# roiponytch/Flickering_Adversarial_Video

Hardware: AMD Instinct MI355X
Metric: attack-iters/sec (I3D 64x224x224, bs=8 per GPU; clip attack-iterations per second, whole job) + 3D-conv TFLOP/s (higher is better)
Workload: dtype bf16; 1 GPU; I3D-RGB flickering attack iteration (1 fwd + 1 dgrad bwd + Adam), 64x224x224 clips, bs=8 per GPU; global_batch=8, frames=64, parallelism=single, collective=none

## Files before the change

flickering_adversarial_video_amd/csrc/pool.hip:

```cpp
#include <stdlib.h>
#include <string.h>
#include "flk_internal.h"
#include "conv_common.h"

#ifdef FLK_ABLATE
#define PF_DBG(bit) (p.dbg & (bit))
#define PG_DBG(bit) (pg.dbg & (bit))
#else
#define PF_DBG(bit) (0)
#define PG_DBG(bit) (0)
#endif

struct PoolKP {
  const char* in; char* out; uint8_t* idx;
  const char* gout; char* gin; const char* mask; const char* add;
  int in_ld, in_coff, out_ld, out_coff, C;
  int gout_ld, gout_coff, gin_ld, gin_coff, mask_ld, mask_coff;
  int B, Ti, Hi, Wi, To, Ho, Wo;
  int kt, kh, kw, st, sh, sw, pt, ph, pw;
  int relu_input;
};

template <typename T> struct PV;
template <> struct PV<bf16_t> {
// ... 793 lines not shown

  frag8 af[KS][2];
  {
    const char* wp = pg.wpack + ((size_t)cslab * KS * 2 * 64 + lane) * 16;
#pragma unroll
    for (int ks = 0; ks < KS; ++ks)
#pragma unroll
      for (int f = 0; f < 2; ++f) af[ks][f] = *(const frag8*)(wp + (size_t)(ks * 2 + f) * 1024);
  }
  auto decode = [&](int hp, size_t& opos, int& lt0, int& lh0, int& lw0) {
    const int a = (int)(((float)hp + 0.5f) * inv_hw), rem = hp - a * nhw;
    const int bq = (int)(((float)rem + 0.5f) * inv_w), c = rem - bq * nw;
    const int ot = o_t0 + a, oh = o_h0 + bq, ow = o_w0 + c;
    opos = (((size_t)(b * k.To + ot) * k.Ho + oh) * k.Wo + ow);
    lt0 = ot * k.st - k.pt - i_t0; lh0 = oh * k.sh - k.ph - i_h0; lw0 = ow * k.sw - k.pw - i_w0;
  };
  auto product = [&](size_t opos, f32x4 (&v)[2]) {
    const char* gp = pg.g + (opos * pg.g_ld + pg.g_coff + q * 8) * 2;
    frag8 bf[KS];
#pragma unroll
    for (int ks = 0; ks < KS; ++ks) bf[ks] = *(const frag8*)(gp + ks * 64);
    v[0] = f32x4{0.f, 0.f, 0.f, 0.f}; v[1] = v[0];
#pragma unroll
    for (int ks = 0; ks < KS; ++ks) {
      v[0] = __builtin_amdgcn_mfma_f32_16x16x32_bf16(af[ks][0], bf[ks], v[0], 0, 0, 0);
      v[1] = __builtin_amdgcn_mfma_f32_16x16x32_bf16(af[ks][1], bf[ks], v[1], 0, 0, 0);
    }
  };
  __syncthreads();
  unsigned mx = 0u;
  for (int base = wave * 16; base < P; base += 64) {
    const int hp = min(base + m, P - 1);
    size_t opos; int lt0, lh0, lw0;
    decode(hp, opos, lt0, lh0, lw0);
    f32x4 v[2];
    product(opos, v);
#pragma unroll
    for (int f = 0; f < 2; ++f)
#pragma unroll
      for (int j = 0; j < 4; ++j) mx = max(mx, __float_as_uint(v[f][j]) & 0x7fffffffu);
  }
#pragma unroll
  for (int off = 32; off > 0; off >>= 1) mx = max(mx, (unsigned)__shfl_xor((int)mx, off));
  if (lane == 0) atomicMax(smax, mx);
  __syncthreads();
  int ex = (int)(*smax >> 23);
  ex = min(max(ex, 26), 254);
  const float scale = __uint_as_float((unsigned)(127 + p.fx_e + 127 - ex) << 23);
  const float inv_scale = __uint_as_float((unsigned)(127 - p.fx_e - 127 + ex) << 23);
  const int khkw = k.kh * k.kw;
  for (int base = wave * 16; base < P; base += 64) {
    const int hp = min(base + m, P - 1);
    const bool live = base + m < P;
    size_t opos; int lt0, lh0, lw0;
    decode(hp, opos, lt0, lh0, lw0);
    unsigned ib[2];
#pragma unroll
    for (int f = 0; f < 2; ++f) ib[f] = *(const unsigned*)(k.idx + opos * k.C + cslab * 32 + f * 16 + q * 4);
    f32x4 v[2];
    product(opos, v);
    if (!live) continue;
#pragma unroll
    for (int f = 0; f < 2; ++f)
#pragma unroll
      for (int j = 0; j < 4; ++j) {
        const int tap = (int)((ib[f] >> (8 * j)) & 255u);
        const int dt = (int)(((unsigned)tap * m_khkw) >> 20), r2 = tap - dt * khkw;
        const int dh = (int)(((unsigned)r2 * m_kw) >> 20), dw = r2 - dh * k.kw;
        const int lt = lt0 + dt, lh = lh0 + dh, lw = lw0 + dw;
        if ((unsigned)lt < (unsigned)p.Tt && (unsigned)lh < (unsigned)p.Ht && (unsigned)lw < (unsigned)p.Wt && dt < k.kt)
          atomicAdd(&acc[(f * 16 + q * 4 + j) * RS + (lt * p.Ht + lh) * p.Wt + lw], (unsigned)__float2int_rn(v[f][j] * scale));
      }
  }
  __syncthreads();
  const int ch = tid & 3, c0 = cslab * 32 + ch * 8;
  if (c0 >= k.C) return;
  const int hw = p.Ht * p.Wt;
  for (int r = tid >> 2; r < p.rows; r += 64) {
    int rt, rh, rw; split3(r, hw, 1.0f / (float)hw, p.Wt, 1.0f / (float)p.Wt, rt, rh, rw);
    const int it = i_t0 + rt, ih = i_h0 + rh, iw = i_w0 + rw;
    if (it >= k.Ti || ih >= k.Hi || iw >= k.Wi) continue;
    float g[8];
#pragma unroll
    for (int e = 0; e < 8; ++e) g[e] = (float)(int)acc[(ch * 8 + e) * RS + r] * inv_scale;
    const size_t ipos = (((size_t)(b * k.Ti + it) * k.Hi + ih) * k.Wi + iw);
    PV<bf16_t>::st(k.gin + (ipos * k.gin_ld + k.gin_coff + c0) * 2, g);
  }
}

template <int KS, int NIT, int NB>
__global__ __launch_bounds__(256, KS >= 3 ? 2 : 3) void maxpool_scatter_gemm_bwd_reg(const PoolGemmP pg, unsigned m_khkw, unsigned m_kw) {
  typedef __bf16 frag8 __attribute__((ext_vector_type(8)));
  extern __shared__ __attribute__((aligned(16))) char smem[];
  unsigned* const acc = (unsigned*)smem;
  const PoolTP& p = pg.t;
  const PoolKP& k = p.k;
  const int RS = p.plane_b;
  const int tid = threadIdx.x, lane = tid & 63, wave = tid >> 6, q = lane >> 4, m = lane & 15;
  int bid, cslab;
  if (!tile_slab_of_block(p, bid, cslab)) return;
  const int tw = bid % p.nTw; bid /= p.nTw;
  const int th = bid % p.nTh; bid /= p.nTh;
  const int tt = bid % p.nTt;
  const int b = bid / p.nTt;
  const int i_t0 = tt * p.Tt, i_h0 = th * p.Ht, i_w0 = tw * p.Wt;
  const int o_t0 = max(0, (i_t0 + k.pt - k.kt + k.st) / k.st), o_t1 = min(k.To - 1, (i_t0 + p.Tt - 1 + k.pt) / k.st);
  const int o_h0 = max(0, (i_h0 + k.ph - k.kh + k.sh) / k.sh), o_h1 = min(k.Ho - 1, (i_h0 + p.Ht - 1 + k.ph) / k.sh);
  const int o_w0 = max(0, (i_w0 + k.pw - k.kw + k.sw) / k.sw), o_w1 = min(k.Wo - 1, (i_w0 + p.Wt - 1 + k.pw) / k.sw);
  const int nt = max(0, o_t1 - o_t0 + 1), nh = max(0, o_h1 - o_h0 + 1), nw = max(0, o_w1 - o_w0 + 1);
  const int nhw = nh * nw, P = nt * nhw;
  const float inv_hw = 1.0f / (float)max(nhw, 1), inv_w = 1.0f / (float)max(nw, 1);
  if (!PG_DBG(16)) for (int i = tid; i < 32 * RS; i += 256) acc[i] = 0u;
  unsigned* const smax = acc + 32 * RS;
  if (tid == 0) *smax = 0u;
  unsigned* const lut = smax + 64;
  {
    const int dt = tid / 9, r2 = tid - dt * 9, dh = r2 / 3, dw = r2 - dh * 3;
    lut[tid] = tid < 27 ? (unsigned)(((dt * p.Ht + dh) * p.Wt + dw) * 4) : 0u;
  }
  f32x4 v[NIT][2];
  unsigned ib[NIT][2];
  int org[NIT];
  unsigned okm[NIT];
  unsigned mx = 0u;
  if (P > 0) {
    frag8 af[KS][2];
    {
      const char* wp = pg.wpack + ((size_t)cslab * KS * 2 * 64 + lane) * 16;
#pragma unroll
      for (int ks = 0; ks < KS; ++ks)
#pragma unroll
        for (int f = 0; f < 2; ++f) af[ks][f] = *(const frag8*)(wp + (size_t)(ks * 2 + f) * 1024);
    }
#pragma unroll
    for (int i0 = 0; i0 < NIT; i0 += NB) {
      frag8 bf[NB][KS];
#pragma unroll
      for (int u = 0; u < NB; ++u) {
        const int i = i0 + u;
        const int hp = wave * 16 + 64 * i + m;
        const bool live = hp < P;
        const int hc = min(hp, P - 1);
        const int a = (int)(((float)hc + 0.5f) * inv_hw), rem = hc - a * nhw;
        const int bq = (int)(((float)rem + 0.5f) * inv_w), c = rem - bq * nw;
        const int ot = o_t0 + a, oh = o_h0 + bq, ow = o_w0 + c;
        const size_t opos = (((size_t)(b * k.To + ot) * k.Ho + oh) * k.Wo + ow);
        const int lt0 = ot * k.st - k.pt - i_t0, lh0 = oh * k.sh - k.ph - i_h0, lw0 = ow * k.sw - k.pw - i_w0;
        org[i] = ((lt0 * p.Ht + lh0) * p.Wt + lw0) * 4;
        auto bits3 = [](int l0, int n) { return (7u << min(max(-l0, 0), 3)) & 7u & ((1u << min(max(n - l0, 0), 3)) - 1u); };
        const unsigned bt3 = bits3(lt0, p.Tt), bh3 = bits3(lh0, p.Ht), bw3 = bits3(lw0, p.Wt);
        const unsigned eh = (bh3 & 1u) | ((bh3 & 2u) << 2) | ((bh3 & 4u) << 4);
        const unsigned et = (bt3 & 1u) | ((bt3 & 2u) << 8) | ((bt3 & 4u) << 16);
        okm[i] = live ? bw3 * eh * et : 0u;
#pragma unroll
        for (int f = 0; f < 2; ++f) ib[i][f] = PG_DBG(8) ? (unsigned)(m * 0x01010101u) & 0x0f0f0f0fu : *(const unsigned*)(k.idx + opos * k.C + cslab * 32 + f * 16 + q * 4);
        const char* gp = pg.g + (opos * pg.g_ld + pg.g_coff + q * 8) * 2;
#pragma unroll
        for (int ks = 0; ks < KS; ++ks) bf[u][ks] = PG_DBG(4) ? af[ks][0] : *(const frag8*)(gp + ks * 64);
      }
#pragma unroll
      for (int u = 0; u < NB; ++u) {
        const int i = i0 + u;
        v[i][0] = f32x4{0.f, 0.f, 0.f, 0.f}; v[i][1] = v[i][0];
#pragma unroll
        for (int ks = 0; ks < KS; ++ks) {
          v[i][0] = __builtin_amdgcn_mfma_f32_16x16x32_bf16(af[ks][0], bf[u][ks], v[i][0], 0, 0, 0);
          v[i][1] = __builtin_amdgcn_mfma_f32_16x16x32_bf16(af[ks][1], bf[u][ks], v[i][1], 0, 0, 0);
        }
#pragma unroll
        for (int f = 0; f < 2; ++f)
#pragma unroll
          for (int j = 0; j < 4; ++j) mx = max(mx, __float_as_uint(v[i][f][j]) & 0x7fffffffu);
      }
    }
  }
#pragma unroll
  for (int off = 32; off > 0; off >>= 1) mx = max(mx, (unsigned)__shfl_xor((int)mx, off));
  __syncthreads();
  if (lane == 0) atomicMax(smax, mx);
  __syncthreads();
  int ex = (int)(*smax >> 23);
  ex = min(max(ex, 26), 254);
  const float scale = __uint_as_float((unsigned)(127 + p.fx_e + 127 - ex) << 23);
  const float inv_scale = __uint_as_float((unsigned)(127 - p.fx_e - 127 + ex) << 23);
  if (P > 0) {
    unsigned* const dummy = lut + 256 + tid;
    if (!PG_DBG(1)) {
#pragma unroll
      for (int i = 0; i < NIT; ++i) {
        char* const plane0 = (char*)acc + (size_t)(q * 4 * RS) * 4 + org[i];
        unsigned off[2][4];
#pragma unroll
        for (int f = 0; f < 2; ++f)
#pragma unroll
          for (int j = 0; j < 4; ++j) off[f][j] = lut[(ib[i][f] >> (8 * j)) & 255u];
        __builtin_amdgcn_sched_barrier(0);
#pragma unroll
        for (int f = 0; f < 2; ++f)
#pragma unroll
          for (int j = 0; j < 4; ++j) {
            const unsigned tap = (ib[i][f] >> (8 * j)) & 255u;
            const bool inside = (okm[i] >> (tap & 31u)) & 1u;
            unsigned* const cell = (unsigned*)(plane0 + (size_t)((f * 16 + j) * RS) * 4 + off[f][j]);
            atomicAdd(inside ? cell : dummy, (unsigned)__float2int_rn(v[i][f][j] * scale));
          }
      }
    }
  }
  __syncthreads();
  const int ch = tid & 3, c0 = cslab * 32 + ch * 8;
  if (c0 >= k.C || PG_DBG(2)) return;
  const int hw = p.Ht * p.Wt;
  for (int r = tid >> 2; r < p.rows; r += 64) {
    int rt, rh, rw; split3(r, hw, 1.0f / (float)hw, p.Wt, 1.0f / (float)p.Wt, rt, rh, rw);
    const int it = i_t0 + rt, ih = i_h0 + rh, iw = i_w0 + rw;
    if (it >= k.Ti || ih >= k.Hi || iw >= k.Wi) continue;
    float g[8];
#pragma unroll
    for (int e = 0; e < 8; ++e) g[e] = (float)(int)acc[(ch * 8 + e) * RS + r] * inv_scale;
    const size_t ipos = (((size_t)(b * k.Ti + it) * k.Hi + ih) * k.Wi + iw);
    PV<bf16_t>::st(k.gin + (ipos * k.gin_ld + k.gin_coff + c0) * 2, g);
  }
}

static flk_tile choose_scatter_tile(const flk_pool_args* a, long max_reach = 0) {
  flk_tile best{1, 1, 1};
  double best_cost = 1e300;
  for (int Tt = 1; Tt <= a->Ti && Tt <= 8; ++Tt)
    for (int Ht = 1; Ht <= a->Hi && Tt * Ht <= 256; ++Ht) {
      const int wmax = 256 / (Tt * Ht) < a->Wi ? 256 / (Tt * Ht) : a->Wi;
      for (int Wt = 1; Wt <= wmax; ++Wt) {
        const double tiles = (double)((a->Ti + Tt - 1) / Tt) * ((a->Hi + Ht - 1) / Ht) * ((a->Wi + Wt - 1) / Wt);
        const double outs = (double)((Tt + a->kt - 2) / a->st + 1) * ((Ht + a->kh - 2) / a->sh + 1) * ((Wt + a->kw - 2) / a->sw + 1);
        if (max_reach > 0 && outs > (double)max_reach) continue;
        const double passes = (double)(((long)outs + 255) / 256);
        const double cost = tiles * (Tt * Ht * Wt * 16.0 + outs * 24.0 + passes * 2048.0 + 2048.0);
        if (cost < best_cost - 1e-9) { best_cost = cost; best = flk_tile{Tt, Ht, Wt}; }
      }
    }
  return best;
}

static int fixed_point_exponent(const flk_pool_args* a) {
  const int n = ((a->kt + a->st - 1) / a->st) * ((a->kh + a->sh - 1) / a->sh) * ((a->kw + a->sw - 1) / a->sw);
  int lg = 0;
  while ((1 << lg) < n) ++lg;
  return 30 - lg < 24 ? 30 - lg : 24;
}

template <typename T>
static int launch_scatter_bwd(const PoolKP& kp, const flk_pool_args* a, hipStream_t s) {
  constexpr int EPL = PV<T>::EPL;
  PoolTP tp{};
  tp.k = kp;
  tp.fx_e = fixed_point_exponent(a);
  const flk_tile t = choose_scatter_tile(a);
  tp.Tt = t.Tt; tp.Ht = t.Ht; tp.Wt = t.Wt; tp.rows = t.Tt * t.Ht * t.Wt;
  tp.nTt = (a->Ti + t.Tt - 1) / t.Tt; tp.nTh = (a->Hi + t.Ht - 1) / t.Ht; tp.nTw = (a->Wi + t.Wt - 1) / t.Wt;
  tp.ntiles = a->B * tp.nTt * tp.nTh * tp.nTw; tp.nslab = (a->C + 4 * EPL - 1) / (4 * EPL);
  const dim3 grid((unsigned)((tp.ntiles + 7) / 8 * 8 * tp.nslab));
  auto magic = [](int d) { return (unsigned)(((1u << 20) + (unsigned)d - 1) / (unsigned)d); };
  tp.plane_b = (tp.rows + 47) / 64 * 64 + 16;
  const size_t lds = (size_t)(4 * tp.plane_b * EPL + 256) * sizeof(float);
  FLK_LAUNCH_KERNEL(maxpool_scatter_bwd<T>, grid, dim3(256), lds, s, tp, magic(a->kh * a->kw), magic(a->kw));
  FLK_CHECK_HIP(hipGetLastError());
  return FLK_OK;
}

static bool use_tiled(const flk_pool_args* a) {
  return a->st == 1 && a->sh == 1 && a->sw == 1 && a->kt * a->kh * a->kw >= 8 && a->To == a->Ti && a->Ho == a->Hi &&
         a->Wo == a->Wi && a->pt < a->kt && a->ph < a->kh && a->pw < a->kw;
}

template <typename T>
static int launch_tiled(const PoolKP& kp, const flk_pool_args* a, bool bwd, hipStream_t s) {
  PoolTP tp{};
  tp.k = kp;
  const flk_tile t = flk_choose_tile(a->To, a->Ho, a->Wo, a->kt, a->kh, a->kw, 1, 1, 1, 256, 768);
  tp.Tt = t.Tt; tp.Ht = t.Ht; tp.Wt = t.Wt; tp.rows = t.Tt * t.Ht * t.Wt;
  tp.nTt = (a->To + t.Tt - 1) / t.Tt; tp.nTh = (a->Ho + t.Ht - 1) / t.Ht; tp.nTw = (a->Wo + t.Wt - 1) / t.Wt;
  tp.Th = t.Tt + a->kt - 1; tp.Hh = t.Ht + a->kh - 1; tp.Wh = t.Wt + a->kw - 1;
  tp.P = tp.Th * tp.Hh * tp.Wh;
  FLK_REQUIRE(tp.P <= FLK_MAX_HALO, "maxpool tiled: halo %d too large", tp.P);
  tp.plane_b = (tp.P * 16 + 255) / 256 * 256;
  constexpr int EPL = PV<T>::EPL;
  const size_t lds = 4 * (size_t)tp.plane_b + 64 + (bwd ? (size_t)4 * tp.P * EPL + 16 : 0);
  tp.ntiles = a->B * tp.nTt * tp.nTh * tp.nTw; tp.nslab = (a->C + 4 * EPL - 1) / (4 * EPL);
  const dim3 grid((unsigned)((tp.ntiles + 7) / 8 * 8 * tp.nslab));
  static bool attr_fwd[FLK_MAX_DEVICES] = {}, attr_bwd[FLK_MAX_DEVICES] = {};
  if (int rc = flk_raise_lds_limit((const void*)maxpool_s1_tiled_fwd<T>, 96 * 1024, attr_fwd)) return rc;
  if (int rc = flk_raise_lds_limit((const void*)maxpool_s1_tiled_bwd<T>, 96 * 1024, attr_bwd)) return rc;
  if (bwd) FLK_LAUNCH_KERNEL(maxpool_s1_tiled_bwd<T>, grid, dim3(256), lds, s, tp);
  else if (sizeof(T) == 2 && a->kt == 3 && a->kh == 3 && a->kw == 3 && a->pt == 1 && a->ph == 1 && a->pw == 1) {
    return a->Wo % 7 == 0 ? launch_wrun_fwd<7>(kp, a, s) : launch_wrun_fwd<8>(kp, a, s);
  } else if (sizeof(T) == 2 && a->kt == 3 && a->kh == 3 && a->kw == 3) {
    static bool attr2[FLK_MAX_DEVICES] = {};
    if (int rc = flk_raise_lds_limit((const void*)maxpool_s1_tiled_fwd_bf16<3, 3, 3>, 96 * 1024, attr2)) return rc;
    FLK_LAUNCH_KERNEL((maxpool_s1_tiled_fwd_bf16<3, 3, 3>), grid, dim3(256), lds, s, tp);
  } else FLK_LAUNCH_KERNEL(maxpool_s1_tiled_fwd<T>, grid, dim3(256), lds, s, tp);
  FLK_CHECK_HIP(hipGetLastError());
  return FLK_OK;
}

static int check_pool(const flk_pool_args* a) {
  FLK_REQUIRE(a && a->in && a->idx, "flk_maxpool3d: null argument");
  FLK_REQUIRE(a->C % 8 == 0 && a->in_ld % 8 == 0 && a->in_coff % 8 == 0 && a->out_ld % 8 == 0 && a->out_coff % 8 == 0,
              "flk_maxpool3d: channel counts / strides / offsets must be multiples of 8");
  FLK_REQUIRE(a->kt * a->kh * a->kw <= 255 && a->kt > 0 && a->kh > 0 && a->kw > 0, "flk_maxpool3d: window too large");
  FLK_REQUIRE(a->B > 0 && a->To > 0 && a->Ho > 0 && a->Wo > 0 && a->st > 0 && a->sh > 0 && a->sw > 0, "flk_maxpool3d: bad dims");
  FLK_REQUIRE(a->pt < a->kt && a->ph < a->kh && a->pw < a->kw &&
                  (a->To - 1) * a->st - a->pt < a->Ti && (a->Ho - 1) * a->sh - a->ph < a->Hi &&
                  (a->Wo - 1) * a->sw - a->pw < a->Wi, "flk_maxpool3d: a window lies entirely in the padding");
  return FLK_OK;
}

static void fill(PoolKP& kp, const flk_pool_args* a) {
  kp.in = (const char*)a->in; kp.out = (char*)a->out; kp.idx = a->idx;
  kp.in_ld = a->in_ld; kp.in_coff = a->in_coff; kp.out_ld = a->out_ld; kp.out_coff = a->out_coff; kp.C = a->C;
  kp.B = a->B; kp.Ti = a->Ti; kp.Hi = a->Hi; kp.Wi = a->Wi; kp.To = a->To; kp.Ho = a->Ho; kp.Wo = a->Wo;
  kp.kt = a->kt; kp.kh = a->kh; kp.kw = a->kw; kp.st = a->st; kp.sh = a->sh; kp.sw = a->sw;
  kp.pt = a->pt; kp.ph = a->ph; kp.pw = a->pw;
  kp.relu_input = a->relu_input;
}

static unsigned grid_for(long total) {
  long g = (total + 255) / 256;
  return (unsigned)(g < 1 ? 1 : (g > 16384 ? 16384 : g));
}

extern "C" int flk_maxpool3d_fwd(const flk_pool_args* a, int dtype, void* stream) {
  int rc = check_pool(a);
  if (rc) return rc;
  FLK_REQUIRE(a->out, "flk_maxpool3d_fwd: null out");
  PoolKP kp{};
  fill(kp, a);
  FLK_REQUIRE(dtype == FLK_BF16 || dtype == FLK_F32, "flk_maxpool3d_fwd: bad dtype");
  if (use_tiled(a)) return dtype == FLK_BF16 ? launch_tiled<bf16_t>(kp, a, false, (hipStream_t)stream) : launch_tiled<float>(kp, a, false, (hipStream_t)stream);
  const int epl = dtype == FLK_BF16 ? 8 : 4;
  FLK_REQUIRE(a->Ho < 65536 && (long)a->B * a->To < 65536, "flk_maxpool3d_fwd: grid too large");
  const dim3 grid((unsigned)((a->Wo * (a->C / epl) + 255) / 256), (unsigned)a->Ho, (unsigned)(a->B * a->To));
  const int kcode = a->kt * 100 + a->kh * 10 + a->kw;
  if (dtype == FLK_BF16) {
    if (kcode == 133) FLK_LAUNCH_KERNEL((maxpool_fwd_kernel_k<bf16_t, 1, 3, 3>), grid, dim3(256), 0, (hipStream_t)stream, kp);
    else if (kcode == 333) FLK_LAUNCH_KERNEL((maxpool_fwd_kernel_k<bf16_t, 3, 3, 3>), grid, dim3(256), 0, (hipStream_t)stream, kp);
    else if (kcode == 222) FLK_LAUNCH_KERNEL((maxpool_fwd_kernel_k<bf16_t, 2, 2, 2>), grid, dim3(256), 0, (hipStream_t)stream, kp);
    else FLK_LAUNCH_KERNEL(maxpool_fwd_kernel<bf16_t>, grid, dim3(256), 0, (hipStream_t)stream, kp);
  } else {
    if (kcode == 133) FLK_LAUNCH_KERNEL((maxpool_fwd_kernel_k<float, 1, 3, 3>), grid, dim3(256), 0, (hipStream_t)stream, kp);
    else if (kcode == 222) FLK_LAUNCH_KERNEL((maxpool_fwd_kernel_k<float, 2, 2, 2>), grid, dim3(256), 0, (hipStream_t)stream, kp);
    else FLK_LAUNCH_KERNEL(maxpool_fwd_kernel<float>, grid, dim3(256), 0, (hipStream_t)stream, kp);
  }
  FLK_CHECK_HIP(hipGetLastError());
  return FLK_OK;
}

extern "C" int flk_maxpool3d_bwd(const flk_pool_args* a, const void* gout, int gout_ld, int gout_coff,
                                 void* gin, int gin_ld, int gin_coff, const void* mask, int mask_ld, int mask_coff,
                                 int dtype, void* stream) {
  int rc = check_pool(a);
  if (rc) return rc;
  FLK_REQUIRE(gout && gin, "flk_maxpool3d_bwd: null gradient");
  FLK_REQUIRE(gout_ld % 8 == 0 && gout_coff % 8 == 0 && gin_ld % 8 == 0 && gin_coff % 8 == 0 && mask_ld % 8 == 0 && mask_coff % 8 == 0,
              "flk_maxpool3d_bwd: ld/coff must be multiples of 8");
  PoolKP kp{};
  fill(kp, a);
  kp.gout = (const char*)gout; kp.gout_ld = gout_ld; kp.gout_coff = gout_coff;
  kp.gin = (char*)gin; kp.gin_ld = gin_ld; kp.gin_coff = gin_coff;
  kp.mask = (const char*)mask; kp.mask_ld = mask_ld; kp.mask_coff = mask_coff;
  kp.add = nullptr;
  FLK_REQUIRE(dtype == FLK_BF16 || dtype == FLK_F32, "flk_maxpool3d_bwd: bad dtype");
  {
    hipStream_t s = (hipStream_t)stream;
#define FLK_OWNER(KT, KH, KW, ST, SH, SW)                                                                   \
    if (strided_owner_ok(a, KT, KH, KW, ST, SH, SW))                                                          \
      return dtype == FLK_BF16 ? launch_strided_bwd<bf16_t, KT, KH, KW, ST, SH, SW>(kp, a, s)                 \
                               : launch_strided_bwd<float, KT, KH, KW, ST, SH, SW>(kp, a, s)
    FLK_OWNER(1, 3, 3, 1, 2, 2); FLK_OWNER(3, 3, 3, 2, 2, 2); FLK_OWNER(2, 2, 2, 2, 2, 2);
#undef FLK_OWNER
  }
  if (dtype == FLK_BF16) return launch_scatter_bwd<bf16_t>(kp, a, (hipStream_t)stream);
  if (use_tiled(a)) return launch_tiled<float>(kp, a, true, (hipStream_t)stream);
  const int epl = dtype == FLK_BF16 ? 8 : 4;
  FLK_REQUIRE(a->Hi < 65536 && (long)a->B * a->Ti < 65536, "flk_maxpool3d_bwd: grid too large");
  const dim3 grid((unsigned)((a->Wi * (a->C / epl) + 255) / 256), (unsigned)a->Hi, (unsigned)(a->B * a->Ti));
  FLK_LAUNCH_KERNEL(maxpool_bwd_kernel<float>, grid, dim3(256), 0, (hipStream_t)stream, kp);
  FLK_CHECK_HIP(hipGetLastError());
  return FLK_OK;
}


extern "C" int flk_pool_gemm_weights_create(const float* wt_kc, int K, int C, void** out_dev) {
  FLK_REQUIRE(wt_kc && out_dev && K > 0 && K % 32 == 0 && K <= 128 && C > 0 && C % 8 == 0, "flk_pool_gemm_weights_create: K must be 32, 64, 96 or 128 and C a multiple of 8 "
              "(got K %d, C %d)", K, C);
  const int nslab = (C + 31) / 32, KS = K / 32;
  std::vector<uint16_t> h((size_t)nslab * KS * 2 * 64 * 8, 0);
  auto bf = [](float f) -> uint16_t {
    uint32_t u; memcpy(&u, &f, 4);
    if ((u & 0x7fffffffu) > 0x7f800000u) return (uint16_t)((u >> 16) | 0x40);
    return (uint16_t)((u + 0x7fffu + ((u >> 16) & 1u)) >> 16);
  };
  for (int s = 0; s < nslab; ++s)
    for (int ks = 0; ks < KS; ++ks)
      for (int f = 0; f < 2; ++f)
        for (int lane = 0; lane < 64; ++lane) {
          const int q = lane >> 4, m = lane & 15, c = s * 32 + f * 16 + m;
          for (int j = 0; j < 8; ++j) {
            const int kk = ks * 32 + q * 8 + j;
            h[((((size_t)s * KS + ks) * 2 + f) * 64 + lane) * 8 + j] = c < C ? bf(wt_kc[(size_t)kk * C + c]) : 0;
          }
        }
  void* d = nullptr;
  hipError_t e = hipMalloc(&d, h.size() * 2);
  if (e != hipSuccess) { flk_set_error("hipMalloc(%zu): %s", h.size() * 2, hipGetErrorString(e)); return FLK_ENOMEM; }
  e = hipMemcpy(d, h.data(), h.size() * 2, hipMemcpyHostToDevice);
  if (e != hipSuccess) { (void)hipFree(d); flk_set_error("hipMemcpy: %s", hipGetErrorString(e)); return FLK_EHIP; }
  *out_dev = d;
  return FLK_OK;
}
extern "C" int flk_pool_gemm_weights_destroy(void* dev) {
  if (dev) (void)hipFree(dev);
  return FLK_OK;
}

extern "C" int flk_maxpool3d_bwd_gemm(const flk_pool_args* a, const void* g, int g_ld, int g_coff, int K, const void* wpack,
                                      void* gin, int gin_ld, int gin_coff, int dtype, void* stream) {
  int rc = check_pool(a);
  if (rc) return rc;
  FLK_REQUIRE(g && wpack && gin, "flk_maxpool3d_bwd_gemm: null argument");
  FLK_REQUIRE(dtype == FLK_BF16, "flk_maxpool3d_bwd_gemm: bf16 only (fp32, the parity mode, keeps the two-launch gather path)");
  FLK_REQUIRE(K > 0 && K % 32 == 0 && K <= 128, "flk_maxpool3d_bwd_gemm: K must be 32, 64, 96 or 128 (got %d)", K);
  FLK_REQUIRE(g_ld % 8 == 0 && g_coff % 8 == 0 && g_coff + K <= g_ld && gin_ld % 8 == 0 && gin_coff % 8 == 0 && gin_coff + a->C <= gin_ld,
              "flk_maxpool3d_bwd_gemm: bad ld / coff");
  FLK_REQUIRE((size_t)a->B * a->To * a->Ho * a->Wo * (size_t)(g_ld > a->C ? g_ld : a->C) < (1ull << 31), "flk_maxpool3d_bwd_gemm: tensor too large");
  PoolGemmP pg{};
  fill(pg.t.k, a);
  pg.t.k.gin = (char*)gin; pg.t.k.gin_ld = gin_ld; pg.t.k.gin_coff = gin_coff;
  pg.g = (const char*)g; pg.g_ld = g_ld; pg.g_coff = g_coff; pg.KS = K / 32; pg.wpack = (const char*)wpack;
#ifdef FLK_ABLATE
  pg.dbg = flk_ablate_env("FLK_PG_DBG");
#endif
  const char* const reg_env = getenv("FLK_POOL_GEMM_REG");
  const bool reg_form = !(reg_env && atoi(reg_env) == 0);
  const bool reg_able = reg_form && a->kt == 3 && a->kh == 3 && a->kw == 3;
  const flk_tile t = choose_scatter_tile(a, reg_able ? 512 : 0);
  PoolTP& tp = pg.t;
  tp.fx_e = fixed_point_exponent(a);
  tp.Tt = t.Tt; tp.Ht = t.Ht; tp.Wt = t.Wt; tp.rows = t.Tt * t.Ht * t.Wt;
  tp.nTt = (a->Ti + t.Tt - 1) / t.Tt; tp.nTh = (a->Hi + t.Ht - 1) / t.Ht; tp.nTw = (a->Wi + t.Wt - 1) / t.Wt;
  tp.ntiles = a->B * tp.nTt * tp.nTh * tp.nTw; tp.nslab = (a->C + 31) / 32;
  const dim3 grid((unsigned)((tp.ntiles + 7) / 8 * 8 * tp.nslab));
  auto magic = [](int d) { return (unsigned)(((1u << 20) + (unsigned)d - 1) / (unsigned)d); };
  {
    constexpr int res = 4;
    tp.plane_b = (tp.rows - res + 63) / 64 * 64 + res;
  }
  const size_t lds = (size_t)(32 * tp.plane_b + 64) * sizeof(float);
  hipStream_t s = (hipStream_t)stream;
  const unsigned m1 = magic(a->kh * a->kw), m2 = magic(a->kw);
  const long reach = (long)((t.Tt + a->kt - 2) / a->st + 1) * ((t.Ht + a->kh - 2) / a->sh + 1) * ((t.Wt + a->kw - 2) / a->sw + 1);
  if (reg_able && reach <= 512) {
    const size_t lds_reg = lds + (size_t)(64 + 256 + 256) * sizeof(unsigned);
    switch (pg.KS) {
      case 1: FLK_LAUNCH_KERNEL((maxpool_scatter_gemm_bwd_reg<1, 8, 4>), grid, dim3(256), lds_reg, s, pg, m1, m2); break;
      case 2: FLK_LAUNCH_KERNEL((maxpool_scatter_gemm_bwd_reg<2, 8, 4>), grid, dim3(256), lds_reg, s, pg, m1, m2); break;
      case 3: FLK_LAUNCH_KERNEL((maxpool_scatter_gemm_bwd_reg<3, 8, 2>), grid, dim3(256), lds_reg, s, pg, m1, m2); break;
      default: FLK_LAUNCH_KERNEL((maxpool_scatter_gemm_bwd_reg<4, 8, 2>), grid, dim3(256), lds_reg, s, pg, m1, m2); break;
    }
    FLK_CHECK_HIP(hipGetLastError());
    return FLK_OK;
  }
  switch (pg.KS) {
    case 1: FLK_LAUNCH_KERNEL(maxpool_scatter_gemm_bwd<1>, grid, dim3(256), lds, s, pg, m1, m2); break;
    case 2: FLK_LAUNCH_KERNEL(maxpool_scatter_gemm_bwd<2>, grid, dim3(256), lds, s, pg, m1, m2); break;
    case 3: FLK_LAUNCH_KERNEL(maxpool_scatter_gemm_bwd<3>, grid, dim3(256), lds, s, pg, m1, m2); break;
    default: FLK_LAUNCH_KERNEL(maxpool_scatter_gemm_bwd<4>, grid, dim3(256), lds, s, pg, m1, m2); break;
  }
  FLK_CHECK_HIP(hipGetLastError());
  return FLK_OK;
}


struct PoolConvFP {
  PoolKP k;
  ConvKP c;
  unsigned npos;
  int write_pool;
};

__global__ __launch_bounds__(256, 3) void maxpool133_conv1x1_fwd(const PoolConvFP p) {
  typedef Prec<bf16_t> PR;
  typedef typename PR::frag frag;
  constexpr int EPL = 8, NF = 4, NTAP = 9, TB = 2;
  extern __shared__ __attribute__((aligned(16))) char smem[];
  const int tid = threadIdx.x, lane = tid & 63;
  const int wave = __builtin_amdgcn_readfirstlane(tid >> 6);
  const int q = lane >> 4, m = lane & 15;
  const PoolKP& k = p.k;
  const unsigned npos = p.npos, pos0 = blockIdx.x * 256u;
  const int gsw[4] = {0, 3, 2, 1};
  {
    const uint4 w0 = *(const uint4*)(p.c.w + tid * 16), w1 = *(const uint4*)(p.c.w + (tid + 256) * 16);
    *(uint4*)(smem + 32768 + tid * 16) = w0;
    *(uint4*)(smem + 32768 + (tid + 256) * 16) = w1;
  }
  const int cg = tid & 7;
  const unsigned hw = (unsigned)(k.Ho * k.Wo);
#pragma unroll 1
  for (int it0 = 0; it0 < 8; it0 += TB) {
    uint4 raw[TB][NTAP];
    bool ok[TB][NTAP];
    unsigned posv[TB];
#pragma unroll
    for (int u = 0; u < TB; ++u) {
      posv[u] = pos0 + (unsigned)((it0 + u) * 32 + (tid >> 3));
      const unsigned pos = posv[u] < npos ? posv[u] : npos - 1;
      const unsigned bt = pos / hw, rem = pos - bt * hw;
      const int oh = (int)(rem / (unsigned)k.Wo), ow = (int)(rem - (unsigned)oh * (unsigned)k.Wo);
#pragma unroll
      for (int dh = 0; dh < 3; ++dh)
#pragma unroll
        for (int dw = 0; dw < 3; ++dw) {
          const int tap = dh * 3 + dw;
          const int ih = oh * 2 - k.ph + dh, iw = ow * 2 - k.pw + dw;
          ok[u][tap] = (unsigned)ih < (unsigned)k.Hi && (unsigned)iw < (unsigned)k.Wi;
          const size_t ipos = ok[u][tap] ? (((size_t)bt * k.Hi + ih) * k.Wi + iw) : 0;
          raw[u][tap] = *(const uint4*)(k.in + (ipos * k.in_ld + k.in_coff + cg * EPL) * 2);
        }
    }
    __builtin_amdgcn_sched_barrier(0);
#pragma unroll
    for (int u = 0; u < TB; ++u) {
      float best[EPL];
      int bi[EPL];
      pool_window_scan<bf16_t, NTAP>(raw[u], ok[u], k.relu_input, best, bi);
      bf16x8 pv;
#pragma unroll
      for (int e = 0; e < EPL; ++e) pv[e] = (bf16_t)best[e];
      if (posv[u] < npos) {
        PV<bf16_t>::stidx(k.idx + (size_t)posv[u] * k.C + cg * EPL, bi);
        if (p.write_pool) *(bf16x8*)(k.out + ((size_t)posv[u] * k.out_ld + k.out_coff + cg * EPL) * 2) = pv;
      }
      const int pl = (it0 + u) * 32 + (tid >> 3);
      *(bf16x8*)(smem + (cg >> 2) * 16384 + pl * 64 + (((cg & 3) ^ gsw[(pl >> 2) & 3]) * 16)) = pv;
    }
  }
  __syncthreads();
  int boff[4];
#pragma unroll
  for (int i = 0; i < 4; ++i) boff[i] = (64 * wave + 16 * i + m) * 64 + ((q ^ gsw[(m >> 2) & 3]) * 16);
  f32x4 acc[NF][4];
#pragma unroll
  for (int f = 0; f < NF; ++f)
#pragma unroll
    for (int i = 0; i < 4; ++i) acc[f][i] = f32x4{0.f, 0.f, 0.f, 0.f};
#pragma unroll
  for (int s = 0; s < 2; ++s) {
    const char* const sb = smem + s * 16384;
    frag bf[4], af[NF];
#pragma unroll
    for (int i = 0; i < 4; ++i) bf[i] = *(const frag*)(sb + boff[i]);
#pragma unroll
    for (int f = 0; f < NF; ++f) af[f] = *(const frag*)(smem + 32768 + ((s * NF + f) * 64 + lane) * 16);
    __builtin_amdgcn_sched_barrier(0);
#pragma unroll
    for (int f = 0; f < NF; ++f)
#pragma unroll
      for (int i = 0; i < 4; ++i) PR::mma(af[f], bf[i], acc[f][i]);
  }
  constexpr int NG = 4 * NF / EPL;
  const int cbase = q * EPL;
  float4 sc[NG][2], bi[NG][2];
  epi_scale_bias_regs<bf16_t, NG>(p.c, cbase, sc, bi);
  uint4 none[NG];
#pragma unroll
  for (int g = 0; g < NG; ++g) none[g] = make_uint4(0u, 0u, 0u, 0u);
#pragma unroll
  for (int i = 0; i < 4; ++i) {
    const unsigned pos = pos0 + (unsigned)(64 * wave + 16 * i + m);
    if (pos >= npos) continue;
    float v[NG][EPL];
#pragma unroll
    for (int g = 0; g < NG; ++g)
#pragma unroll
      for (int e = 0; e < EPL; ++e) v[g][e] = acc[(g * EPL + e) >> 2][i][(g * EPL + e) & 3];
    finish_store_row_ops<bf16_t, NG>(p.c, (size_t)pos, nullptr, cbase, v, sc, bi, none, none);
  }
}

struct PoolConvBP {
  PoolKP k;
  const char* w;
  const char* g;
  char* gp;
  int g_ld, g_coff, gp_ld, gp_coff;
  int Hb, Wb, lgWb, nTh, nTw;
};
constexpr int POOL_CONV_BWD_MAXFRAG = 20;

__global__ __launch_bounds__(256, 3) void maxpool133_conv1x1_bwd(const PoolConvBP p) {
  typedef Prec<bf16_t> PR;
  typedef typename PR::frag frag;
  constexpr int EPL = 8;
  extern __shared__ __attribute__((aligned(16))) char smem[];
  const int tid = threadIdx.x, lane = tid & 63;
  const int wave = __builtin_amdgcn_readfirstlane(tid >> 6);
  const int q = lane >> 4, m = lane & 15;
  const PoolKP& k = p.k;
  int bid = blockIdx.x;
  const int tw = bid % p.nTw; bid /= p.nTw;
  const int th = bid % p.nTh;
  const int bt = bid / p.nTh;
  const int b = bt / k.To, ot = bt - b * k.To;
  const int oh0 = th * p.Hb, ow0 = tw * p.Wb;
  const int Wp = p.Wb + 1, P = (p.Hb + 1) * Wp, nfrag = (P + 15) >> 4;
  const int cg = tid & 7;

  auto task_window = [&](int it, int& wh, int& ww) {
    const int wl = it * 32 + (tid >> 3);
    wh = wl >> p.lgWb; ww = wl & (p.Wb - 1);
    return oh0 + wh < k.Ho && ow0 + ww < k.Wo;
  };
  auto load_idx = [&](int it, uint2 (&r)[4]) {
    int wh, ww;
    if (!task_window(it, wh, ww)) { r[0] = r[1] = r[2] = r[3] = make_uint2(0u, 0u); return; }
    const int oh = oh0 + wh, ow = ow0 + ww;
#pragma unroll
    for (int dh = 0; dh < 2; ++dh)
#pragma unroll
      for (int dw = 0; dw < 2; ++dw) {
        const size_t opos = ((size_t)bt * k.Ho + max(oh - dh, 0)) * k.Wo + max(ow - dw, 0);
        r[dh * 2 + dw] = *(const uint2*)(k.idx + opos * k.C + cg * EPL);
      }
  };
  uint2 ia[4][4];
#pragma unroll
  for (int it = 0; it < 4; ++it) load_idx(it, ia[it]);

  {
    frag af[2][4];
#pragma unroll
// ... 154 lines not shown
```

Measured before the change: 1536 clip-iters/s.

## Add temporal-column maxpool kernel for 3x3x3 stride-2 bf16 pooling

Adds a dedicated forward maxpool kernel for 3x3x3 stride-2 bf16 windows. Each thread walks a column of output frames along time and reuses the shared input plane between adjacent temporal windows, so each plane is loaded about once instead of up to twice. Loads of the next plane are double-buffered against the reduction. The frames per thread are picked from a wave-count heuristic. This trades parallelism, since there are fewer threads each doing serial work, for less redundant global memory traffic. An env var can force or disable the path.

After: 1543 clip-iters/s, median of 6. Within noise of the previous version (+0.5%).

```diff
diff --git a/flickering_adversarial_video_amd/csrc/pool.hip b/flickering_adversarial_video_amd/csrc/pool.hip
--- a/flickering_adversarial_video_amd/csrc/pool.hip
+++ b/flickering_adversarial_video_amd/csrc/pool.hip
@@ -1119,6 +1119,100 @@
   return FLK_OK;
 }
 
+__global__ __launch_bounds__(256) void maxpool333s2_tcol_fwd_bf16(const PoolKP p, int TC, int nTc) {
+  constexpr int EPL = 8;
+  const int ng = p.C / EPL;
+  const unsigned i = blockIdx.x * 256u + threadIdx.x;
+  if (i >= (unsigned)(p.Ho * p.Wo * ng)) return;
+  const int oh = i / (p.Wo * ng), r = i - oh * (p.Wo * ng), ow = r / ng, cg = r - ow * ng;
+  const int tc = blockIdx.y % nTc, b = blockIdx.y / nTc;
+  const int ot0 = tc * TC, nout = min(TC, p.To - ot0);
+  bool okhw[9];
+  int off[9];
+#pragma unroll
+  for (int dh = 0; dh < 3; ++dh)
+#pragma unroll
+    for (int dw = 0; dw < 3; ++dw) {
+      const int ih = oh * 2 - p.ph + dh, iw = ow * 2 - p.pw + dw;
+      okhw[dh * 3 + dw] = (unsigned)ih < (unsigned)p.Hi && (unsigned)iw < (unsigned)p.Wi;
+      off[dh * 3 + dw] = okhw[dh * 3 + dw] ? ih * p.Wi + iw : 0;
+    }
+  const char* const base = p.in + (size_t)(p.in_coff + cg * EPL) * 2;
+  const int it0 = ot0 * 2 - p.pt;
+  auto load_plane = [&](int q, uint4 (&raw)[9]) {
+    const size_t pl = (size_t)(b * p.Ti + ((unsigned)(it0 + q) < (unsigned)p.Ti ? it0 + q : 0)) * p.Hi * p.Wi;
+#pragma unroll
+    for (int j = 0; j < 9; ++j) raw[j] = *(const uint4*)(base + (pl + off[j]) * p.in_ld * 2);
+  };
+  float best[EPL], pv[EPL];
+  int bi[EPL], pi[EPL];
+  auto reduce = [&](int q, const uint4 (&raw)[9]) {
+    const bool okt = (unsigned)(it0 + q) < (unsigned)p.Ti;
+    bool ok[9];
+#pragma unroll
+    for (int j = 0; j < 9; ++j) ok[j] = okhw[j] && okt;
+    pool_window_scan<bf16_t, 9>(raw, ok, 0, pv, pi);
+  };
+  auto fold = [&](int dt) {
+#pragma unroll
+    for (int e = 0; e < EPL; ++e)
+      if (pv[e] > best[e]) { best[e] = pv[e]; bi[e] = pi[e] + 9 * dt; }
+  };
+  auto open_window = [&]() {
+#pragma unroll
+    for (int e = 0; e < EPL; ++e) { best[e] = -INFINITY; bi[e] = 0; }
+    fold(0);
+  };
+  uint4 ra[9], rb[9];
+  load_plane(0, rb);
+  load_plane(1, ra);
+  reduce(0, rb);
+  open_window();
+#pragma unroll 1
+  for (int j = 0; j < nout; ++j) {
+    load_plane(2 * j + 2, rb);
+    reduce(2 * j + 1, ra);
+    fold(1);
+    if (j + 1 < nout) load_plane(2 * j + 3, ra);
+    reduce(2 * j + 2, rb);
+    fold(2);
+    if (p.relu_input) {
+#pragma unroll
+      for (int e = 0; e < EPL; ++e) bi[e] = best[e] > 0.f ? bi[e] : 255;
+    }
+    const size_t opos = (((size_t)(b * p.To + ot0 + j) * p.Ho + oh) * p.Wo + ow);
+    PV<bf16_t>::st(p.out + (opos * p.out_ld + p.out_coff + cg * EPL) * 2, best);
+    PV<bf16_t>::stidx(p.idx + opos * p.C + cg * EPL, bi);
+    open_window();
+  }
+}
+
+static int launch_pool4a_tcol(const PoolKP& kp, const flk_pool_args* a, int TC, hipStream_t s) {
+  const int nTc = (a->To + TC - 1) / TC;
+  const long per = (long)a->Ho * a->Wo * (a->C / 8);
+  FLK_REQUIRE(per < (1l << 31) - 256 && (long)a->B * nTc < 65536 && (long)a->Hi * a->Wi < (1l << 30), "flk_maxpool3d_fwd: grid too large");
+  const dim3 grid((unsigned)((per + 255) / 256), (unsigned)(a->B * nTc));
+  FLK_LAUNCH_KERNEL(maxpool333s2_tcol_fwd_bf16, grid, dim3(256), 0, s, kp, TC, nTc);
+  flk_last_kernel_tag = "maxpool333s2_tcol_fwd_bf16";
+  FLK_CHECK_HIP(hipGetLastError());
+  return FLK_OK;
+}
+
+static int pool4a_switch() { static const int v = getenv("FLK_POOL_TILED_4A") ? atoi(getenv("FLK_POOL_TILED_4A")) : 1; return v; }
+
+static bool pool4a_tcol_ok(const flk_pool_args* a, int dtype) {
+  return pool4a_switch() != 0 && dtype == FLK_BF16 && a->kt == 3 && a->kh == 3 && a->kw == 3 && a->st == 2 && a->sh == 2 && a->sw == 2;
+}
+
+static int pool4a_frames_per_thread(const flk_pool_args* a) {
+  const int forced = pool4a_switch();
+  if (forced == 2 || forced == 4 || forced == 8) return forced;
+  const long waves = ((long)a->B * a->Ho * a->Wo * (a->C / 8) + 63) / 64;
+  for (int tc = 8; tc > 2; tc >>= 1)
+    if (waves * ((a->To + tc - 1) / tc) >= 2048) return tc;
+  return 2;
+}
+
 static int check_pool(const flk_pool_args* a) {
   FLK_REQUIRE(a && a->in && a->idx, "flk_maxpool3d: null argument");
   FLK_REQUIRE(a->C % 8 == 0 && a->in_ld % 8 == 0 && a->in_coff % 8 == 0 && a->out_ld % 8 == 0 && a->out_coff % 8 == 0,
@@ -1153,6 +1247,7 @@
   fill(kp, a);
   FLK_REQUIRE(dtype == FLK_BF16 || dtype == FLK_F32, "flk_maxpool3d_fwd: bad dtype");
   if (use_tiled(a)) return dtype == FLK_BF16 ? launch_tiled<bf16_t>(kp, a, false, (hipStream_t)stream) : launch_tiled<float>(kp, a, false, (hipStream_t)stream);
+  if (pool4a_tcol_ok(a, dtype)) return launch_pool4a_tcol(kp, a, pool4a_frames_per_thread(a), (hipStream_t)stream);
   const int epl = dtype == FLK_BF16 ? 8 : 4;
   FLK_REQUIRE(a->Ho < 65536 && (long)a->B * a->To < 65536, "flk_maxpool3d_fwd: grid too large");
   const dim3 grid((unsigned)((a->Wo * (a->C / epl) + 255) / 256), (unsigned)a->Ho, (unsigned)(a->B * a->To));
```
